# CompVis/zigma

Hardware: NVIDIA H100
Metric: denoiser tokens/s (bs*L*evals/s), zigzag8_b1, Euler sampling loop (higher is better)
Workload: dtype bf16

## Files before the change

include/zigma_b200.h:

```cpp
#ifndef ZIGMA_B200_H
#define ZIGMA_B200_H

#include <stdint.h>

#ifdef __cplusplus
extern "C" {
#endif

enum { ZG_F32 = 0, ZG_F16 = 1, ZG_BF16 = 2 };

enum {
    ZG_SCAN_DELTA_SOFTPLUS = 1,
    ZG_SCAN_VARIABLE_B = 2,
    ZG_SCAN_VARIABLE_C = 4,
    ZG_SCAN_OUT_REVERSE = 8,
    ZG_SCAN_OUT_ACCUMULATE = 16
};

int zg_abi_version(void);
const char *zg_last_error(void);
uint64_t zg_launch_count(void);
const char *zg_last_scan_kernel(void);
int zg_scan_kernel_choice(int64_t units16, int32_t sms, int32_t training_forward, int32_t *nd, int32_t *ns);

// ... 104 lines not shown
    const float *d_residual_out;
    const void *d_normed, *d_modded;
    const float *r, *rstd;
    const void *mix, *gate, *scale, *norm_w;
    const int32_t *rowmap;
    void *d_x, *d_mix;
    float *d_residual_in, *dgate, *dshift, *dscale, *d_norm_w;
    int64_t mod_rs;
    int32_t batch, seqlen, dim, dtype, nparts;
} zg_block_tail_bwd_params;

int zg_block_tail_bwd(const zg_block_tail_bwd_params *p, void *stream);

int64_t zg_selective_scan_bwd_det_workspace_bytes(const zg_scan_bwd_params *p);
int zg_selective_scan_bwd_det(const zg_scan_bwd_params *p, void *workspace, int64_t workspace_bytes, void *stream);
int64_t zg_causal_conv1d_bwd_det_workspace_bytes(const zg_conv_bwd_params *p);
int zg_causal_conv1d_bwd_det(const zg_conv_bwd_params *p, void *workspace, int64_t workspace_bytes, void *stream);
int64_t zg_add_norm_bwd_det_workspace_bytes(const zg_norm_bwd_params *p);
int zg_add_norm_bwd_det(const zg_norm_bwd_params *p, void *workspace, int64_t workspace_bytes, void *stream);
int64_t zg_block_tail_bwd_det_workspace_bytes(const zg_block_tail_bwd_params *p);
int zg_block_tail_bwd_det(const zg_block_tail_bwd_params *p, void *workspace, int64_t workspace_bytes, void *stream);

typedef struct {
    zg_block_tail_params base;
    const void *path_scale;
} zg_block_tail_dp_params;

typedef struct {
    zg_block_tail_bwd_params base;
    const void *path_scale;
} zg_block_tail_bwd_dp_params;

int zg_block_tail_fwd_dp(const zg_block_tail_dp_params *p, void *stream);
int zg_block_tail_bwd_dp(const zg_block_tail_bwd_dp_params *p, void *stream);
int64_t zg_block_tail_bwd_dp_det_workspace_bytes(const zg_block_tail_bwd_dp_params *p);
int zg_block_tail_bwd_dp_det(const zg_block_tail_bwd_dp_params *p, void *workspace, int64_t workspace_bytes, void *stream);

typedef struct {
    const void *q, *k, *v;
    void *o;
    float *lse;
    int64_t q_sb, q_rs, k_sb, k_rs, v_sb, v_rs, o_sb, o_rs;
    int32_t batch, L, Lk, heads, dim, dtype;
} zg_xattn_params;

int zg_cross_attn_fwd(const zg_xattn_params *p, void *stream);

typedef struct {
    zg_xattn_params fwd;
    const void *dout;
    void *dq, *dk, *dv;
    int64_t dout_sb, dout_rs, dq_sb, dq_rs, dk_sb, dk_rs, dv_sb, dv_rs;
    int32_t sms;
} zg_xattn_bwd_params;

int64_t zg_cross_attn_bwd_workspace_bytes(const zg_xattn_bwd_params *p);
int zg_cross_attn_bwd(const zg_xattn_bwd_params *p, void *workspace, int64_t workspace_bytes, void *stream);

typedef struct {
    const void *A, *B, *bias;
    void *C;
    const int32_t *out_rowmap;
    int64_t lda, ldb, ldc;
    int32_t M, N, K, rows_per_batch;
} zg_gemm_params;

// ... 44 lines not shown
```

zigma_b200/_lib.py:

```python
import ctypes as C
import os

import torch

_HERE = os.path.dirname(os.path.abspath(__file__))
LIB_PATH = os.environ.get("ZIGMA_B200_LIB") or os.path.join(_HERE, "lib", "libzigma_b200.so")

ZG_F32, ZG_F16, ZG_BF16 = 0, 1, 2
SCAN_DELTA_SOFTPLUS, SCAN_VARIABLE_B, SCAN_VARIABLE_C, SCAN_OUT_REVERSE, SCAN_OUT_ACCUMULATE = 1, 2, 4, 8, 16
_DT = {torch.float32: ZG_F32, torch.float16: ZG_F16, torch.bfloat16: ZG_BF16}

vp, i64, i32, f32 = C.c_void_p, C.c_int64, C.c_int32, C.c_float


class ScanParams(C.Structure):
    _fields_ = ([(n, vp) for n in ("u", "delta", "z", "B", "C", "A", "D", "delta_bias", "z_rowmap", "out", "last_state", "ckpt")]
                + [(n, i64) for n in ("u_sb", "u_sd", "u_sl", "delta_sb", "delta_sd", "delta_sl", "z_sb", "z_sd", "z_sl",
                                      "out_sb", "out_sd", "out_sl", "B_sb", "B_sg", "B_sn", "B_sl", "C_sb", "C_sg", "C_sn", "C_sl")]
                + [(n, i32) for n in ("batch", "dim", "seqlen", "dstate", "ngroups", "dtype", "flags", "ckpt_every")]
                + [(n, vp) for n in ("dt_w", "dt_x")]
                + [(n, i64) for n in ("dt_w_ld", "dt_x_sb", "dt_x_sl")]
                + [(n, i32) for n in ("dt_rank", "z_batch_inner")]
                + [("z_sbi", i64)])

# ... 25 lines not shown
                + [(n, i64) for n in ("x_rs", "res_rs", "y_rs", "resout_rs")]
                + [(n, i32) for n in ("nrows", "ncols", "dtype", "res_dtype", "wdtype", "is_rms")]
                + [("eps", f32)])


class NormBwdParams(C.Structure):
    _fields_ = ([(n, vp) for n in ("dy", "dresidual", "x", "weight", "mean", "rstd", "dx", "dresidual_in", "dweight", "dbias")]
                + [(n, i64) for n in ("dy_rs", "dres_rs", "x_rs", "dx_rs", "dresin_rs")]
                + [(n, i32) for n in ("nrows", "ncols", "dtype", "res_dtype", "wdtype", "is_rms")])


class BlockTailParams(C.Structure):
    _fields_ = ([(n, vp) for n in ("x", "mix", "gate", "shift", "scale", "norm_w", "residual", "rowmap", "residual_out", "normed", "modded")]
                + [("mod_rs", i64)]
                + [(n, i32) for n in ("batch", "seqlen", "dim", "dtype", "final_layer")]
                + [("eps", f32), ("rstd", vp)])


class BlockTailBwdParams(C.Structure):
    _fields_ = ([(n, vp) for n in ("d_residual_out", "d_normed", "d_modded", "r", "rstd", "mix", "gate", "scale", "norm_w", "rowmap",
                                   "d_x", "d_mix", "d_residual_in", "dgate", "dshift", "dscale", "d_norm_w")]
                + [("mod_rs", i64)]
                + [(n, i32) for n in ("batch", "seqlen", "dim", "dtype", "nparts")])


class BlockTailDpParams(C.Structure):
    _fields_ = [("base", BlockTailParams), ("path_scale", vp)]


class BlockTailBwdDpParams(C.Structure):
    _fields_ = [("base", BlockTailBwdParams), ("path_scale", vp)]


class XattnParams(C.Structure):
    _fields_ = ([(n, vp) for n in ("q", "k", "v", "o", "lse")]
                + [(n, i64) for n in ("q_sb", "q_rs", "k_sb", "k_rs", "v_sb", "v_rs", "o_sb", "o_rs")]
                + [(n, i32) for n in ("batch", "L", "Lk", "heads", "dim", "dtype")])


class XattnBwdParams(C.Structure):
    _fields_ = ([("fwd", XattnParams)]
                + [(n, vp) for n in ("dout", "dq", "dk", "dv")]
                + [(n, i64) for n in ("dout_sb", "dout_rs", "dq_sb", "dq_rs", "dk_sb", "dk_rs", "dv_sb", "dv_rs")]
                + [("sms", i32)])


class TextPrologueParams(C.Structure):
    _fields_ = ([(n, vp) for n in ("x", "mix", "gate", "shift", "scale", "rowmap", "hidden", "q_in", "mean", "rstd")]
                + [("mod_rs", i64)]
                + [(n, i32) for n in ("batch", "seqlen", "dim", "dtype")]
                + [("eps", f32)])


class TextPrologueBwdParams(C.Structure):
    _fields_ = ([(n, vp) for n in ("d_hidden", "d_q", "hidden", "mix", "gate", "scale", "mean", "rstd", "rowmap", "d_x", "d_mix",
                                   "dgate", "dshift", "dscale")]
                + [("mod_rs", i64)]
                + [(n, i32) for n in ("batch", "seqlen", "dim", "dtype", "nparts")])


class GemmParams(C.Structure):
    _fields_ = ([(n, vp) for n in ("A", "B", "bias", "C", "out_rowmap")]
                + [(n, i64) for n in ("lda", "ldb", "ldc")]
                + [(n, i32) for n in ("M", "N", "K", "rows_per_batch")])


class AdamWParams(C.Structure):
    _fields_ = ([(n, vp) for n in ("param", "exp_avg", "exp_avg_sq", "ema", "grad", "grad_scale_ptr")]
                + [("n", i64)]
                + [(n, f32) for n in ("lr", "beta1", "beta2", "eps", "weight_decay", "bias_correction1", "bias_correction2",
                                      "ema_decay", "grad_scale")])


EXPORTS = ["zg_abi_version", "zg_last_error", "zg_launch_count", "zg_last_scan_kernel", "zg_scan_kernel_choice", "zg_selective_scan_fwd", "zg_selective_scan_bwd",
           "zg_causal_conv1d_fwd", "zg_causal_conv1d_bwd", "zg_add_norm_fwd", "zg_add_norm_bwd",
           "zg_block_tail_fwd", "zg_block_tail_fwd_pe", "zg_block_tail_bwd", "zg_block_tail_fwd_dp", "zg_block_tail_bwd_dp",
           "zg_gemm_bf16_tn", "zg_adamw_ema_step", "zg_text_prologue_fwd", "zg_text_prologue_bwd"]
DET_OPS = ["zg_selective_scan_bwd", "zg_causal_conv1d_bwd", "zg_add_norm_bwd", "zg_block_tail_bwd", "zg_block_tail_bwd_dp",
           "zg_text_prologue_bwd"]
EXPORTS += [n + s for n in DET_OPS for s in ("_det", "_det_workspace_bytes")]
EXPORTS += ["zg_cross_attn_fwd", "zg_cross_attn_bwd", "zg_cross_attn_bwd_workspace_bytes"]

_lib = None


def lib():
    global _lib
    if _lib is None:
        if not os.path.exists(LIB_PATH):
            raise RuntimeError(
                f"zigma_b200: native library {LIB_PATH} not found -- build it with "
                f"`python -c 'import __graft_entry__ as g; g.build()'` (nvcc, sm_90a). There is no CPU/PyTorch fallback.")
        l = C.CDLL(LIB_PATH)
        l.zg_last_error.restype = C.c_char_p
        l.zg_launch_count.restype = C.c_uint64
        l.zg_last_scan_kernel.restype = C.c_char_p
        l.zg_last_scan_kernel.argtypes = []
        l.zg_scan_kernel_choice.restype = C.c_int
        l.zg_scan_kernel_choice.argtypes = [C.c_int64, C.c_int32, C.c_int32, C.POINTER(C.c_int32), C.POINTER(C.c_int32)]
        for name in EXPORTS[5:]:
            if name.endswith("_det_workspace_bytes"):
                getattr(l, name).restype = C.c_int64
                getattr(l, name).argtypes = [C.c_void_p]
            elif name.endswith("_det"):
                getattr(l, name).restype = C.c_int
                getattr(l, name).argtypes = [C.c_void_p, C.c_void_p, C.c_int64, C.c_void_p]
            else:
                getattr(l, name).restype = C.c_int
                getattr(l, name).argtypes = [C.c_void_p, C.c_void_p]
# ... 61 lines not shown
```

zigma_b200/csrc/norm.cu:

```cuda
#include "zg_common.cuh"
#include <stdlib.h>

namespace zg {

__device__ __forceinline__ float ld_dt(const void *p, int64_t i, int dt) {
    if (dt == ZG_F32) return reinterpret_cast<const float *>(p)[i];
    if (dt == ZG_F16) return __half2float(reinterpret_cast<const __half *>(p)[i]);
    return __bfloat162float(reinterpret_cast<const __nv_bfloat16 *>(p)[i]);
}
__device__ __forceinline__ void st_dt(void *p, int64_t i, int dt, float v) {
    if (dt == ZG_F32) reinterpret_cast<float *>(p)[i] = v;
    else if (dt == ZG_F16) reinterpret_cast<__half *>(p)[i] = __float2half_rn(v);
    else reinterpret_cast<__nv_bfloat16 *>(p)[i] = __float2bfloat16_rn(v);
}
template <typename T> __device__ __forceinline__ float round_to(float v) { return zg_to_float<T>(zg_from_float<T>(v)); }

template <typename T> __device__ __forceinline__ void ld4(const T *p, int64_t i, float (&o)[4]);
template <> __device__ __forceinline__ void ld4<float>(const float *p, int64_t i, float (&o)[4]) {
    float4 v = *reinterpret_cast<const float4 *>(p + i);
    o[0] = v.x; o[1] = v.y; o[2] = v.z; o[3] = v.w;
}
template <> __device__ __forceinline__ void ld4<__nv_bfloat16>(const __nv_bfloat16 *p, int64_t i, float (&o)[4]) {
    uint2 v = *reinterpret_cast<const uint2 *>(p + i);
    o[0] = __uint_as_float(v.x << 16); o[1] = __uint_as_float(v.x & 0xffff0000u);
// ... 342 lines not shown
            if (q < nq) {
                float o[4];
#pragma unroll
                for (int i = 0; i < 4; ++i) o[i] = (r[k][i] - mean) * rstd2;
                st4<T>(normed, 4 * q, o);
            }
        }
        return;
    }
#pragma unroll
    for (int k = 0; k < MAXQ; ++k) {
        const int q = lane + 32 * k;
        if (q < nq) {
            st4<T>(normed, 4 * q, r[k]);
            if (modded) {
                float sc[4], sh[4], o[4];
                ld4<T>(scale, 4 * q, sc);
                ld4<T>(shift, 4 * q, sh);
#pragma unroll
                for (int i = 0; i < 4; ++i)
                    o[i] = round_to<T>(r[k][i] * round_to<T>(1.f + sc[i])) + sh[i];
                st4<T>(modded, 4 * q, o);
            }
        }
    }
}

#ifndef ZG_TAIL_PREFETCH_MOD
#define ZG_TAIL_PREFETCH_MOD 1
#endif
#ifndef ZG_TAIL_MINB
#define ZG_TAIL_MINB 12
#endif
template <typename T, int MAXQ, bool PE, bool DP>
__device__ __forceinline__ void block_tail_row4_body(const zg_block_tail_params &p, const void *path_scale) {
    __shared__ float red[3][4];
    const int64_t row = blockIdx.x;
    const int tid = threadIdx.x, lane = tid & 31, warp = tid >> 5;
    const int D = p.dim, nq = D >> 2;
    const int b = (int)(row / p.seqlen), l = (int)(row % p.seqlen);
    const T *x = reinterpret_cast<const T *>(p.x) + row * D;
    const T *mix = nullptr;
    if (p.mix) {
        const int64_t src = (PE ? 0 : (int64_t)b * p.seqlen) + (p.rowmap ? p.rowmap[l] : l);
        mix = reinterpret_cast<const T *>(p.mix) + src * D;
    }
    const T *gate = (!PE && p.gate) ? reinterpret_cast<const T *>(p.gate) + (int64_t)b * p.mod_rs : nullptr;
    const T *shift = p.shift ? reinterpret_cast<const T *>(p.shift) + (int64_t)b * p.mod_rs : nullptr;
    const T *scale = p.scale ? reinterpret_cast<const T *>(p.scale) + (int64_t)b * p.mod_rs : nullptr;
    const T *nw = reinterpret_cast<const T *>(p.norm_w);
    const float *res = p.residual ? p.residual + row * D : nullptr;
    float *rout = p.residual_out ? p.residual_out + row * D : nullptr;
    T *normed = reinterpret_cast<T *>(p.normed) + row * D;
    T *modded = p.modded ? reinterpret_cast<T *>(p.modded) + row * D : nullptr;
    auto block_sum = [&](float v, int slot) {
        v = zg_warp_sum(v);
        if (lane == 0) red[slot][warp] = v;
        __syncthreads();
        return (red[slot][0] + red[slot][1]) + (red[slot][2] + red[slot][3]);
    };

    Raw4<T> rx[MAXQ], rm[MAXQ], rg[MAXQ], rw[MAXQ];
#if ZG_TAIL_PREFETCH_MOD
    Raw4<T> rsc[MAXQ], rsh[MAXQ];
#endif
    float4 rr[MAXQ];
#pragma unroll
    for (int k = 0; k < MAXQ; ++k) {
        const int q = tid + 128 * k;
        if (q < nq) {
            rx[k] = ldraw<T>(x, 4 * q);
            if (mix) { rm[k] = ldraw<T>(mix, 4 * q); rg[k] = PE ? raw_ones<T>() : ldraw<T>(gate, 4 * q); }
            if (res) rr[k] = *reinterpret_cast<const float4 *>(res + 4 * q);
            rw[k] = ldraw<T>(nw, 4 * q);
#if ZG_TAIL_PREFETCH_MOD
            if (modded) { rsc[k] = ldraw<T>(scale, 4 * q); rsh[k] = ldraw<T>(shift, 4 * q); }
#endif
        }
    }
    float dps = 1.f;
    if constexpr (DP) dps = zg_to_float<T>(reinterpret_cast<const T *>(path_scale)[b]);
    float r[MAXQ][4];
    float sumsq = 0.f;
#pragma unroll
    for (int k = 0; k < MAXQ; ++k) {
        const int q = tid + 128 * k;
        if (q < nq) {
            cvt4<T>(rx[k], r[k]);
            if (mix) {
                float m[4], g[4];
                cvt4<T>(rm[k], m);
                cvt4<T>(rg[k], g);
#pragma unroll
                for (int i = 0; i < 4; ++i)
                    r[k][i] = round_to<T>(r[k][i] + round_to<T>(g[i] * m[i]));
            }
            if constexpr (DP) {
#pragma unroll
                for (int i = 0; i < 4; ++i) r[k][i] = round_to<T>(__fmul_rn(r[k][i], dps));
            }
            if (res) {
                r[k][0] += rr[k].x; r[k][1] += rr[k].y; r[k][2] += rr[k].z; r[k][3] += rr[k].w;
            }
            if (rout) st4<float>(rout, 4 * q, r[k]);
#pragma unroll
            for (int i = 0; i < 4; ++i) sumsq += r[k][i] * r[k][i];
        }
    }
    const float rstd = 1.f / sqrtf(block_sum(sumsq, 0) / D + p.eps);
    if (p.rstd && tid == 0) p.rstd[row] = rstd;
    float sum2 = 0.f;
#pragma unroll
    for (int k = 0; k < MAXQ; ++k) {
        const int q = tid + 128 * k;
        if (q < nq) {
            float w[4];
            cvt4<T>(rw[k], w);
#pragma unroll
            for (int i = 0; i < 4; ++i) {
                r[k][i] = round_to<T>(r[k][i] * rstd * w[i]);
                sum2 += r[k][i];
            }
        }
    }
    if (!DP && p.final_layer) {
        const float mean = block_sum(sum2, 1) / D;
        float s2 = 0.f;
#pragma unroll
        for (int k = 0; k < MAXQ; ++k)
            if (tid + 128 * k < nq)
#pragma unroll
                for (int i = 0; i < 4; ++i) { const float d = r[k][i] - mean; s2 += d * d; }
        const float rstd2 = 1.f / sqrtf(block_sum(s2, 2) / D + 1e-6f);
#pragma unroll
        for (int k = 0; k < MAXQ; ++k) {
            const int q = tid + 128 * k;
            if (q < nq) {
                float o[4];
#pragma unroll
                for (int i = 0; i < 4; ++i) o[i] = (r[k][i] - mean) * rstd2;
                st4<T>(normed, 4 * q, o);
            }
        }
        return;
    }
#pragma unroll
    for (int k = 0; k < MAXQ; ++k) {
        const int q = tid + 128 * k;
        if (q < nq) {
            st4<T>(normed, 4 * q, r[k]);
            if (modded) {
                float sc[4], sh[4], o[4];
#if ZG_TAIL_PREFETCH_MOD
                cvt4<T>(rsc[k], sc);
                cvt4<T>(rsh[k], sh);
#else
                ld4<T>(scale, 4 * q, sc);
                ld4<T>(shift, 4 * q, sh);
#endif
#pragma unroll
                for (int i = 0; i < 4; ++i)
                    o[i] = round_to<T>(r[k][i] * round_to<T>(1.f + sc[i])) + sh[i];
                st4<T>(modded, 4 * q, o);
            }
        }
    }
}

template <typename T, int MAXQ, bool PE>
__global__ void __launch_bounds__(128, ZG_TAIL_MINB) block_tail_row4_kernel(const zg_block_tail_params p) {
    block_tail_row4_body<T, MAXQ, PE, false>(p, nullptr);
}

template <typename T, int MAXQ>
__global__ void __launch_bounds__(128, ZG_TAIL_MINB) block_tail_dp_fwd_kernel(const zg_block_tail_dp_params p) {
    block_tail_row4_body<T, MAXQ, false, true>(p.base, p.path_scale);
}

template <typename T> static int block_tail_dp_t(const zg_block_tail_dp_params &p, cudaStream_t s) {
    const unsigned g4 = (unsigned)((int64_t)p.base.batch * p.base.seqlen);
    if (p.base.dim <= 512) block_tail_dp_fwd_kernel<T, 1><<<g4, 128, 0, s>>>(p);
    else block_tail_dp_fwd_kernel<T, 2><<<g4, 128, 0, s>>>(p);
    zg_count_launch();
    return zg_check_launch("block_tail_fwd_dp");
}

template <typename T> static int block_tail_t(const zg_block_tail_params &p, cudaStream_t s, bool pe = false) {
    const int64_t nrows = (int64_t)p.batch * p.seqlen;
    static int row4 = -1;
    if (row4 < 0) { const char *e = getenv("ZG_TAIL_ROW4"); row4 = e ? atoi(e) : 1; }
    if ((row4 || pe) && nrows <= 0x7fffffffLL && p.dim <= 2048) {
        const unsigned g4 = (unsigned)nrows;
#define ZG_TAIL4(Q) do { if (pe) block_tail_row4_kernel<T, Q, true><<<g4, 128, 0, s>>>(p); else block_tail_row4_kernel<T, Q, false><<<g4, 128, 0, s>>>(p); } while (0)
        if (p.dim <= 512) ZG_TAIL4(1);
        else if (p.dim <= 1024) ZG_TAIL4(2);
        else if (p.dim <= 1536) ZG_TAIL4(3);
        else ZG_TAIL4(4);
#undef ZG_TAIL4
        zg_count_launch();
        return zg_check_launch("block_tail_fwd");
    }
    if (pe) return zg_set_error("block_tail_fwd_pe: dim <= 2048 and fewer than 2^31 rows only, got dim %d", p.dim);
    const unsigned grid = (unsigned)((nrows * 32 + 127) / 128);
    if (p.dim <= 512) block_tail_kernel<T, 4><<<grid, 128, 0, s>>>(p);
    else if (p.dim <= 640) block_tail_kernel<T, 5><<<grid, 128, 0, s>>>(p);
    else if (p.dim <= 768) block_tail_kernel<T, 6><<<grid, 128, 0, s>>>(p);
    else if (p.dim <= 1024) block_tail_kernel<T, 8><<<grid, 128, 0, s>>>(p);
    else if (p.dim <= 1536) block_tail_kernel<T, 12><<<grid, 128, 0, s>>>(p);
    else block_tail_kernel<T, NORM_MAXQ><<<grid, 128, 0, s>>>(p);
// ... 345 lines not shown
    if (pp->nrows == 0) return 0;
    return norm_bwd_dispatch<false>(*pp, (cudaStream_t)stream);
}

static ZgDetLayout norm_bwd_det_layout(const zg_norm_bwd_params &p, void *ws) {
    ZgDetLayout lay;
    lay.ws = static_cast<unsigned char *>(ws);
    if (p.nrows <= 0 || p.ncols <= 0) return lay;
    const int64_t rows = (int64_t)zg::norm_bwd_grid(p) * (zg::norm_bwd_vec(p) ? 1 : 4);
    lay.add(p.dweight, rows, p.ncols);
    lay.add(p.dbias, rows, p.ncols);
    return lay;
}

extern "C" int64_t zg_add_norm_bwd_det_workspace_bytes(const zg_norm_bwd_params *p) {
    return p ? norm_bwd_det_layout(*p, nullptr).bytes : 0;
}

extern "C" int zg_add_norm_bwd_det(const zg_norm_bwd_params *pp, void *workspace, int64_t workspace_bytes, void *stream) {
    ZG_REQUIRE(pp != nullptr, "add_norm_bwd_det: null params");
    if (int rc = norm_bwd_validate(*pp)) return rc;
    if (pp->nrows == 0) return 0;
    const ZgDetLayout lay = norm_bwd_det_layout(*pp, workspace);
    ZG_REQUIRE_WORKSPACE(lay, workspace, workspace_bytes, "add_norm_bwd_det");
    zg_norm_bwd_params p = *pp;
    int i = 0;
    if (p.dweight) p.dweight = lay.reg[i++].part;
    if (p.dbias) p.dbias = lay.reg[i++].part;
    cudaStream_t s = (cudaStream_t)stream;
    if (int rc = norm_bwd_dispatch<true>(p, s)) return rc;
    return lay.reduce(s);
}

static int block_tail_fwd_validate(const zg_block_tail_params &p, bool pe) {
    ZG_REQUIRE(p.x && p.norm_w && p.normed, "block_tail_fwd: null tensor pointer");
    if (pe) ZG_REQUIRE(p.mix && !p.gate && !p.rowmap && !p.residual, "block_tail_fwd_pe: takes the (seqlen, dim) table as mix and no gate / rowmap / residual");
    else ZG_REQUIRE(!p.mix || p.gate, "block_tail_fwd: mix needs gate");
    ZG_REQUIRE(!p.modded || (p.shift && p.scale), "block_tail_fwd: modded needs shift and scale");
    ZG_REQUIRE(p.dim > 0 && p.dim % 4 == 0 && p.dim <= 4 * 32 * zg::NORM_MAXQ, "block_tail_fwd: dim must be a multiple of 4 and <= %d, got %d",
               4 * 32 * zg::NORM_MAXQ, p.dim);
    ZG_REQUIRE(p.mod_rs % 4 == 0, "block_tail_fwd: modulation row stride must be a multiple of 4");
    ZG_REQUIRE(aligned16(p.x) && aligned16(p.mix) && aligned16(p.residual) && aligned16(p.residual_out) && aligned16(p.normed) && aligned16(p.modded),
               "block_tail_fwd: row tensors must be 16-byte aligned");
    ZG_REQUIRE(aligned_quad(p.gate, p.dtype) && aligned_quad(p.shift, p.dtype) && aligned_quad(p.scale, p.dtype) && aligned_quad(p.norm_w, p.dtype),
               "block_tail_fwd: gate / shift / scale / norm_w must be aligned to 4 elements");
    return 0;
}

static int block_tail_fwd_entry(const zg_block_tail_params *pp, void *stream, bool pe) {
    ZG_REQUIRE(pp != nullptr, "block_tail_fwd: null params");
    const zg_block_tail_params &p = *pp;
    if (int rc = block_tail_fwd_validate(p, pe)) return rc;
    const int64_t nrows = (int64_t)p.batch * p.seqlen;
    if (nrows == 0) return 0;
    cudaStream_t s = (cudaStream_t)stream;
    switch (p.dtype) {
        case ZG_F32: return zg::block_tail_t<float>(p, s, pe);
        case ZG_F16: return zg::block_tail_t<__half>(p, s, pe);
        case ZG_BF16: return zg::block_tail_t<__nv_bfloat16>(p, s, pe);
    }
    return zg_set_error("block_tail_fwd: bad dtype %d", p.dtype);
}

extern "C" int zg_block_tail_fwd(const zg_block_tail_params *pp, void *stream) { return block_tail_fwd_entry(pp, stream, false); }
extern "C" int zg_block_tail_fwd_pe(const zg_block_tail_params *pp, void *stream) { return block_tail_fwd_entry(pp, stream, true); }

static bool aligned_elem(const void *p, int dtype) {
    return (reinterpret_cast<uintptr_t>(p) & ((dtype == ZG_F32 ? sizeof(float) : sizeof(__half)) - 1)) == 0;
}

extern "C" int zg_block_tail_fwd_dp(const zg_block_tail_dp_params *pp, void *stream) {
    ZG_REQUIRE(pp != nullptr, "block_tail_fwd_dp: null params");
    const zg_block_tail_params &p = pp->base;
    ZG_REQUIRE(pp->path_scale != nullptr, "block_tail_fwd_dp: null path_scale");
    ZG_REQUIRE(p.residual != nullptr && p.mix != nullptr, "block_tail_fwd_dp: needs residual and mix (the first block has no drop path)");
    ZG_REQUIRE(p.final_layer == 0, "block_tail_fwd_dp: final_layer is not supported");
    ZG_REQUIRE(p.dim <= 1024, "block_tail_fwd_dp: dim must be <= 1024, got %d", p.dim);
    if (int rc = block_tail_fwd_validate(p, false)) return rc;
    ZG_REQUIRE(aligned_elem(pp->path_scale, p.dtype), "block_tail_fwd_dp: path_scale must be aligned to its element size");
    const int64_t nrows = (int64_t)p.batch * p.seqlen;
    if (nrows == 0) return 0;
    ZG_REQUIRE(nrows <= 0x7fffffffLL, "block_tail_fwd_dp: fewer than 2^31 rows only");
    cudaStream_t s = (cudaStream_t)stream;
    switch (p.dtype) {
        case ZG_F32: return zg::block_tail_dp_t<float>(*pp, s);
        case ZG_F16: return zg::block_tail_dp_t<__half>(*pp, s);
        case ZG_BF16: return zg::block_tail_dp_t<__nv_bfloat16>(*pp, s);
    }
    return zg_set_error("block_tail_fwd_dp: bad dtype %d", p.dtype);
}

static int block_tail_bwd_validate(const zg_block_tail_bwd_params &p) {
    ZG_REQUIRE(p.r && p.rstd && p.norm_w && p.d_x, "block_tail_bwd: null tensor pointer");
    ZG_REQUIRE((p.mix != nullptr) == (p.gate != nullptr) && (p.mix != nullptr) == (p.d_mix != nullptr), "block_tail_bwd: mix, gate and d_mix go together");
    ZG_REQUIRE(!p.d_modded || p.scale, "block_tail_bwd: d_modded needs scale");
    ZG_REQUIRE(p.dim > 0 && p.dim % 4 == 0 && p.dim <= 1024, "block_tail_bwd: dim must be a multiple of 4 and <= 1024, got %d", p.dim);
    ZG_REQUIRE(p.mod_rs % 4 == 0, "block_tail_bwd: modulation row stride must be a multiple of 4");
    ZG_REQUIRE(p.nparts >= 1 && p.nparts <= 65535, "block_tail_bwd: nparts (rows of the d_norm_w partials buffer = CTAs) must be in [1, 65535]");
    ZG_REQUIRE(p.dtype == ZG_F32 || p.dtype == ZG_F16 || p.dtype == ZG_BF16, "block_tail_bwd: bad dtype %d", p.dtype);
    ZG_REQUIRE(aligned16(p.r) && aligned16(p.d_residual_out) && aligned16(p.d_normed) && aligned16(p.d_modded) && aligned16(p.mix) && aligned16(p.d_x) &&
                   aligned16(p.d_mix) && aligned16(p.d_residual_in),
// ... 170 lines not shown
```

zigma_b200/csrc/scan_fwd_wp2.cuh:

```cuda
#pragma once
#include "scan_fwd_wp.cuh"

namespace zg {

constexpr int WP2_CH = 32;
constexpr int WP2_MAX_WARPS = 9;

struct Wp2Layout {
    static constexpr int NSTAGE = 3;
    static constexpr int TILE = PT_TL * WP2_CH * 2;
    static constexpr int RAW = 3 * TILE + PT_TL * 64;
    static constexpr int DDU_ROW = WP2_CH * 8;
    static constexpr int DDU_OFF = NSTAGE * RAW;
    static constexpr int BCF_OFF = DDU_OFF + PT_TL * DDU_ROW;
    static constexpr int BAR_OFF = BCF_OFF + PT_TL * 32 * 4;
    static constexpr int WARP_BYTES = ((BAR_OFF + NSTAGE * 8 + 127) / 128) * 128;
};

template <int PITCH>
__device__ __forceinline__ void wp2_main_stage(const unsigned char *__restrict__ ddu_j, const float *__restrict__ bq, unsigned char *__restrict__ ypart,
                                               zg_f2 (&h)[2][4], const zg_f2 (&Al)[2][4]) {
    auto decay = [&](float dlx, const zg_f2 (&al)[4], zg_f2 (&a)[4]) {
        const zg_f2 dl = zg_splat2(dlx);
#pragma unroll
        for (int q = 0; q < 4; ++q) a[q] = zg_ex2_mufu2(zg_mul2(dl, al[q]));
    };
    zg_f2 a0[4], a1[4];
    float4 dd = *reinterpret_cast<const float4 *>(ddu_j);
    decay(dd.x, Al[0], a0);
    decay(dd.z, Al[1], a1);
#pragma unroll
    for (int t = 0; t < PT_TL; ++t) {
        const float4 *bc = reinterpret_cast<const float4 *>(bq + t * 16);
        zg_f2 Bp[4], Cp[4];
#pragma unroll
        for (int k = 0; k < 2; ++k) {
            const float4 Bk = bc[32 * k], Ck = bc[2 + 32 * k];
            Bp[2 * k] = make_float2(Bk.x, Bk.y); Bp[2 * k + 1] = make_float2(Bk.z, Bk.w);
            Cp[2 * k] = make_float2(Ck.x, Ck.y); Cp[2 * k + 1] = make_float2(Ck.z, Ck.w);
// ... 143 lines not shown
    int slot = 0, nslot = 1;
    uint32_t npar = 0;
    for (int s = 0; s < nstages; ++s) {
        wp2_main_stage<LY::DDU_ROW>(ddu_j, bq, ypart, h2, Al2p);
        const unsigned char *raw = smem + slot * LY::RAW;
        __syncwarp();
        if (s + 1 < nstages) {
            const unsigned char *rawn = smem + nslot * LY::RAW;
            zg_mbar_wait(&full[nslot], npar);
#pragma unroll
            for (int k = 0; k < NITEM; ++k) { post_item(k, raw); pre_item(k, rawn); }
            bc_convert(rawn);
        } else {
#pragma unroll
            for (int k = 0; k < NITEM; ++k) post_item(k, raw);
        }
        gout += out_stage;
        __syncwarp();
        issue_stage(slot);
        slot = nslot;
        if (++nslot == NSTAGE) { nslot = 0; npar ^= 1; }
    }
    if (p.last_state) {
#pragma unroll
        for (int c = 0; c < 2; ++c) {
            float4 *dst = reinterpret_cast<float4 *>(p.last_state + ((int64_t)b * E + e + c) * 16 + 8 * part);
            dst[0] = make_float4(h2[c][0].x, h2[c][0].y, h2[c][1].x, h2[c][1].y);
            dst[1] = make_float4(h2[c][2].x, h2[c][2].y, h2[c][3].x, h2[c][3].y);
        }
    }
}

template <typename T, bool PLAIN>
__global__ void __launch_bounds__(32 * WP2_MAX_WARPS, 2) scan_fwd_wp2_kernel(const zg_scan_params p) {
    extern __shared__ __align__(1024) unsigned char smem_all[];
    const int lane = threadIdx.x & 31;
    const int warp = __shfl_sync(0xffffffffu, (int)(threadIdx.x >> 5), 0);
    const int per_group = p.dim / p.ngroups;
    const int units_per_group = per_group / WP2_CH;
    const int units = units_per_group * p.ngroups;
    const int wu = blockIdx.x * (int)(blockDim.x >> 5) + warp;
    if (wu >= units * p.batch) return;
    const int unit = wu % units;
    wp2_body<T, PLAIN>(p, smem_all + warp * Wp2Layout::WARP_BYTES, lane, wu / units, unit / units_per_group, unit * WP2_CH);
}

inline int wp2_pick_warps(long long units, int sms) {
    if (units > 18LL * sms) return 3;
    const long long per_sm = (units + sms - 1) / sms;
    const int ctas_per_sm = per_sm > 4 ? 2 : 1;
    return (int)((units + (long long)sms * ctas_per_sm - 1) / ((long long)sms * ctas_per_sm));
}

template <typename T, bool PLAIN> int wp2_launch(const zg_scan_params &p, cudaStream_t stream) {
    using LY = Wp2Layout;
    auto kern = scan_fwd_wp2_kernel<T, PLAIN>;
    static bool attr_dev[64] = {};
    static int sms_dev[64] = {};
    int dev = 0;
    cudaGetDevice(&dev);
    if (!attr_dev[dev & 63]) {
        cudaError_t err = cudaFuncSetAttribute(kern, cudaFuncAttributeMaxDynamicSharedMemorySize, WP2_MAX_WARPS * LY::WARP_BYTES);
        if (err != cudaSuccess) return zg_set_error("scan_fwd(wp2): cudaFuncSetAttribute(%d B smem): %s", WP2_MAX_WARPS * LY::WARP_BYTES, cudaGetErrorString(err));
        cudaFuncSetAttribute(kern, cudaFuncAttributePreferredSharedMemoryCarveout, cudaSharedmemCarveoutMaxShared);
        cudaDeviceGetAttribute(&sms_dev[dev & 63], cudaDevAttrMultiProcessorCount, dev);
        attr_dev[dev & 63] = true;
    }
    const long long units = (long long)(p.dim / WP2_CH) * p.batch;
    const int w = wp2_pick_warps(units, sms_dev[dev & 63] > 0 ? sms_dev[dev & 63] : 132);
    const long long nblk = (units + w - 1) / w;
    kern<<<(unsigned)nblk, 32 * w, w * LY::WARP_BYTES, stream>>>(p);
    zg_count_launch();
    zg_note_scan_kernel("zg::scan_fwd_wp2_kernel (warp-private pipeline, 32 channels per warp, cp.async)");
    return zg_check_launch("scan_fwd(wp2)");
}

template <typename T> int wp2_launch_variant(const zg_scan_params &p, cudaStream_t stream) {
    const bool plain = p.z && (p.flags & ZG_SCAN_DELTA_SOFTPLUS) && !(p.flags & (ZG_SCAN_OUT_REVERSE | ZG_SCAN_OUT_ACCUMULATE));
    return plain ? wp2_launch<T, true>(p, stream) : wp2_launch<T, false>(p, stream);
}

}
```

zigma_b200/engine.py:

```python
import os

import torch
import torch.nn.functional as F

from . import _lib
from .causal_conv1d_interface import _conv_fwd
from .selective_scan_interface import _scan_fwd


def _i32(t):
    return t.to(torch.int32).contiguous()


def _linear(x2d, weight, bias=None):
    if x2d.dtype == torch.bfloat16 and os.environ.get("ZIGMA_TCGEN05", "1") == "1" and x2d.stride(0) % 8 == 0 and weight.stride(0) % 8 == 0:
        from .gemm import linear_bf16
        return linear_bf16(x2d, weight, bias)
    return F.linear(x2d, weight, bias)


def fused_dt_ok(dtype, E, L, N, R, dt_w):
    return (dtype in (torch.bfloat16, torch.float16) and N == 16 and R in (40, 48) and L % 8 == 0 and E % 64 == 0
            and dt_w.dtype == dtype and dt_w.stride(1) == 1 and dt_w.stride(0) % 8 == 0 and (R + 2 * N) % 8 == 0)


def scan_hot_path_ok(dtype, E, L, N, R):
    return (dtype in (torch.bfloat16, torch.float16) and N == 16 and L % 8 == 0 and L > 0 and E % 64 == 0 and R % 8 == 0
            and (R + 2 * N) % 8 == 0 and os.environ.get("ZG_SCAN_TMA", "1") != "0")


def block_tail(x, mix, gate, shift, scale, norm_w, residual, rowmap, eps, final=False, mod_div=1, want_modded=True, want_rstd=False,
               mix_bcast=False, path_scale=None):
    _lib.require_cuda(x, mix, gate, shift, scale, norm_w, residual, rowmap, path_scale)
    if path_scale is not None and (path_scale.dtype != x.dtype or tuple(path_scale.shape) != (x.shape[0],) or not path_scale.is_contiguous()):
        raise RuntimeError(f"block_tail: path_scale must be a contiguous ({x.shape[0]},) tensor in {x.dtype}, got "
                           f"{tuple(path_scale.shape)} {path_scale.dtype}")
    Bt, L, D = x.shape
    if mod_div != 1:
        gate = None if gate is None else gate.repeat_interleave(mod_div, dim=0)
        shift = None if shift is None else shift.repeat_interleave(mod_div, dim=0)
        scale = None if scale is None else scale.repeat_interleave(mod_div, dim=0)
    mods = [m for m in (gate, shift, scale) if m is not None]
    rs = mods[0].stride(0) if mods else 0
    for m in mods:
        if m.stride(0) != rs or m.stride(1) != 1:
            raise RuntimeError("block_tail: modulation views must share one row stride")
    if norm_w.dtype != x.dtype:
        norm_w = norm_w.to(x.dtype)
    def _as_x(t):
        return t if (t is None or t.dtype == x.dtype) else t.to(x.dtype)
    mix = _as_x(mix)
    if mix is not None and not mix.is_contiguous():
        mix = mix.contiguous()
    if any(m is not None and m.dtype != x.dtype for m in (gate, shift, scale)):
        D_ = x.shape[-1]
        packed = torch.zeros((x.shape[0] // mod_div if mod_div != 1 else x.shape[0], 3 * D_), dtype=x.dtype, device=x.device)
        for i_, m in enumerate((gate, shift, scale)):
            if m is not None:
                packed[:, i_ * D_:(i_ + 1) * D_] = m
        gate = None if gate is None else packed[:, :D_]
        shift = None if shift is None else packed[:, D_:2 * D_]
        scale = None if scale is None else packed[:, 2 * D_:]
    if residual is not None and residual.dtype != torch.float32:
        raise RuntimeError("block_tail: the residual stream must be fp32 (residual_in_fp32=True)")
    res_out = torch.empty((Bt, L, D), dtype=torch.float32, device=x.device) if not final else None
    normed = torch.empty_like(x)
    modded = torch.empty_like(x) if (want_modded and not final) else None
    p = _lib.BlockTailParams()
    p.x, p.mix, p.gate, p.shift, p.scale = _lib.ptr(x), _lib.ptr(mix), _lib.ptr(gate), _lib.ptr(shift), _lib.ptr(scale)
    p.norm_w, p.residual, p.rowmap = _lib.ptr(norm_w), _lib.ptr(residual), _lib.ptr(rowmap)
    p.residual_out, p.normed, p.modded = _lib.ptr(res_out), _lib.ptr(normed), _lib.ptr(modded)
    p.mod_rs = rs
    p.batch, p.seqlen, p.dim = Bt, L, D
    p.dtype, p.final_layer, p.eps = _lib.dt(x), int(final), float(eps)
    rstd = torch.empty((Bt * L,), dtype=torch.float32, device=x.device) if want_rstd else None
    p.rstd = _lib.ptr(rstd)
    if mix_bcast and (mix is None or mix.numel() != L * D or gate is not None or rowmap is not None or residual is not None):
        raise RuntimeError("block_tail: mix_bcast takes a (seqlen, dim) mix table and no gate / rowmap / residual")
    if path_scale is not None:
        _lib.call("zg_block_tail_fwd_dp", _lib.BlockTailDpParams(p, _lib.ptr(path_scale)))
    else:
        _lib.call("zg_block_tail_fwd_pe" if mix_bcast else "zg_block_tail_fwd", p)
    if want_rstd:
        return res_out, normed, modded, rstd
    return res_out, normed, modded


def text_prologue(x, mix, gate, shift, scale, rowmap, eps, mod_div=1, want_stats=False):
    _lib.require_cuda(x, mix, gate, shift, scale, rowmap)
    Bt, L, D = x.shape
    if mod_div != 1:
        gate, shift, scale = (m.repeat_interleave(mod_div, dim=0) for m in (gate, shift, scale))
    if any(t.dtype != x.dtype for t in (mix, gate, shift, scale)) or tuple(mix.shape) != (Bt, L, D) or not mix.is_contiguous():
        raise RuntimeError("text_prologue: mix must be a contiguous tensor of x's shape and every operand in x's dtype")
    rs = gate.stride(0)
    if any(m.stride(0) != rs or m.stride(1) != 1 or tuple(m.shape) != (Bt, D) for m in (gate, shift, scale)):
        raise RuntimeError("text_prologue: gate / shift / scale must be (batch, dim) views sharing one row stride")
    hidden, q_in = torch.empty_like(x), torch.empty_like(x)
    mean = torch.empty((Bt * L,), dtype=torch.float32, device=x.device) if want_stats else None
    rstd = torch.empty((Bt * L,), dtype=torch.float32, device=x.device) if want_stats else None
    p = _lib.TextPrologueParams()
    p.x, p.mix, p.gate, p.shift, p.scale, p.rowmap = _lib.ptr(x), _lib.ptr(mix), _lib.ptr(gate), _lib.ptr(shift), _lib.ptr(scale), _lib.ptr(rowmap)
    p.hidden, p.q_in, p.mean, p.rstd = _lib.ptr(hidden), _lib.ptr(q_in), _lib.ptr(mean), _lib.ptr(rstd)
    p.mod_rs = rs
    p.batch, p.seqlen, p.dim, p.dtype, p.eps = Bt, L, D, _lib.dt(x), float(eps)
    _lib.call("zg_text_prologue_fwd", p)
    if want_stats:
        return hidden, q_in, mean, rstd
    return hidden, q_in


class ZigMaEngine:
# ... 157 lines not shown
                y = self._core(xz, B * T, K, lay, lay["fwd"], lay["perm"])
                mix = _linear(y.reshape(B * T * K, E), lay["out_proj"], lay["out_bias"]).view(B * T, K, D)
                return mix, lay["perm_rev"], T
            if self._temporal_fused_ok(xz.dtype, lay, T, K):
                tb = self._temporal_tables(lay, T, K, xz.device)
                y = self._core_temporal(xz, B, T, K, lay, lay["fwd"], tb)
                mix = _linear(y.reshape(B * L, E), lay["out_proj"], lay["out_bias"]).view(B, L, D)
                return mix, tb["out"], 1
            xz_t = xz.view(B, T, K, 2 * E).permute(0, 2, 1, 3).reshape(B * K * T, 2 * E)
            y = self._core(xz_t, B * K, T, lay, lay["fwd"], lay["perm"])
            mix = _linear(y.reshape(B * K * T, E), lay["out_proj"], lay["out_bias"]).view(B * K, T, D)
            mix = mix[:, lay["perm_rev64"], :].reshape(B, K, T, D).permute(0, 2, 1, 3).reshape(B, L, D)
            return mix, None, 1
        mix = _linear(y.reshape(B * L, E), lay["out_proj"], lay["out_bias"]).view(B, L, D)
        return mix, rowmap, 1

    def _forward_impl(self, x, t, y):
        m = self.m
        tokens = self._patch_embed(x)
        pe = None
        if (tokens is not None and m.use_pe in (1, 2) and not (m.video_frames > 0 and m.tpe) and m.pos_embed.dtype == tokens.dtype
                and tokens.shape[-1] <= 2048 and os.environ.get("ZIGMA_FOLD_PE", "1") != "0"):
            pe = m.pos_embed.detach().reshape(-1, m.pos_embed.shape[-1]).contiguous()
        hs, c, text = m.embed(x, t, y, tokens=tokens, add_pos=pe is None)
        hs = hs.contiguous()
        B, L, D = hs.shape
        if pe is not None and pe.shape[0] != L:
            raise RuntimeError(f"pos_embed has {pe.shape[0]} rows, the model {L} tokens")
        depth = len(self.layers)
        nmod = 6 if m.has_text else 3
        mods = _linear(F.silu(c), self.ada_w, self.ada_b).view(B, depth, nmod, D)
        eps = m.blocks[0].norm.eps
        lay0 = self.layers[0]
        residual, normed, modded = block_tail(hs, pe, None, mods[:, 0, 0], mods[:, 0, 1], lay0["norm_w"], None, None, eps,
                                              mix_bcast=pe is not None)
        for i, lay in enumerate(self.layers):
            mix, rowmap, fold = self._mixer(modded, lay)
            last = i == depth - 1
            nw = m.norm_f.weight if last else self.layers[i + 1]["norm_w"]
            neps = m.norm_f.eps if last else m.blocks[i + 1].norm.eps
            gate = mods[:, i, 2]
            shift = None if last else mods[:, i + 1, 0]
            scale = None if last else mods[:, i + 1, 1]
            if m.has_text:
                blk = m.blocks[i]
                Bf = B * fold
                hidden, q_in = text_prologue(normed.view(Bf, L // fold, D), mix.view(Bf, L // fold, D), gate, mods[:, i, 3], mods[:, i, 4],
                                             rowmap, blk.norm_msa.eps, mod_div=fold)
                fold = 1
                mix, rowmap, gate, normed = blk.msa(q_in.view(B, L, D), text=text, mask=None).contiguous(), None, mods[:, i, 5], hidden.view(B, L, D)
            if fold != 1:
                Bf = B * fold
                residual, normed, modded = block_tail(normed.view(Bf, L // fold, D), mix, gate, shift, scale, nw,
                                                      residual.view(Bf, L // fold, D), rowmap, neps, final=last, mod_div=fold)
                normed = normed.view(B, L, D)
                if not last:
                    residual, modded = residual.view(B, L, D), modded.view(B, L, D)
            else:
                residual, normed, modded = block_tail(normed, mix, gate, shift, scale, nw, residual, rowmap, neps, final=last)
        out = _linear(normed.reshape(B * L, D), m.final_layer.linear.weight, m.final_layer.linear.bias).view(B, L, -1)
        if m.video_frames > 0:
            return m.unpatchify_video(out, m.video_frames)
        return m.unpatchify(out)

    @torch.no_grad()
    def forward(self, x, t, y=None):
        if self._versions != self._param_versions():
            self.refresh()
        if not self.use_graph:
            return self._forward_impl(x, t, y)
        key = (tuple(x.shape), x.dtype, tuple(t.shape), t.dtype, None if y is None else (tuple(y.shape), y.dtype))
        g = self._graphs.get(key)
        if g is None:
            sx, st_, sy = x.clone(), t.clone(), None if y is None else y.clone()
            s = torch.cuda.Stream()
            s.wait_stream(torch.cuda.current_stream())
            with torch.cuda.stream(s):
                for _ in range(2):
                    self._forward_impl(sx, st_, sy)
            torch.cuda.current_stream().wait_stream(s)
            graph = torch.cuda.CUDAGraph()
            with torch.cuda.graph(graph):
                sout = self._forward_impl(sx, st_, sy)
            g = (graph, sx, st_, sy, sout)
            self._graphs[key] = g
        graph, sx, st_, sy, sout = g
        sx.copy_(x)
        st_.copy_(t)
        if y is not None:
            sy.copy_(y)
        graph.replay()
        return sout.clone()
# ... 53 lines not shown
```

Measured before the change: 2.166 million.

## Rebuild normed input from residual and rstd in block tail; widen scan warps

Adds a block-tail variant that recomputes the previous layer's normed activations from the fp32 residual, the per-row rstd and the norm weight, instead of writing and re-reading a bf16 normed tensor. Intermediate normed outputs are no longer stored, which removes one activation write and read per layer. Separately, the wp2 scan kernel now allows up to 20 warps per CTA with one CTA per SM, and the warp-count heuristic changes to match, spreading small workloads across more warps. The cost is an extra rstd write per row and some recompute work, plus different occupancy and register limits in the scan kernel.

```diff
diff --git a/include/zigma_b200.h b/include/zigma_b200.h
--- a/include/zigma_b200.h
+++ b/include/zigma_b200.h
@@ -160,6 +160,14 @@
 } zg_block_tail_bwd_dp_params;
 
 int zg_block_tail_fwd_dp(const zg_block_tail_dp_params *p, void *stream);
+
+typedef struct {
+    zg_block_tail_params base;
+    const float *x_rstd;
+    const void *x_norm_w;
+} zg_block_tail_rebuild_params;
+
+int zg_block_tail_fwd_rebuild(const zg_block_tail_rebuild_params *p, void *stream);
 int zg_block_tail_bwd_dp(const zg_block_tail_bwd_dp_params *p, void *stream);
 int64_t zg_block_tail_bwd_dp_det_workspace_bytes(const zg_block_tail_bwd_dp_params *p);
 int zg_block_tail_bwd_dp_det(const zg_block_tail_bwd_dp_params *p, void *workspace, int64_t workspace_bytes, void *stream);
diff --git a/zigma_b200/_lib.py b/zigma_b200/_lib.py
--- a/zigma_b200/_lib.py
+++ b/zigma_b200/_lib.py
@@ -81,6 +81,10 @@
     _fields_ = [("base", BlockTailBwdParams), ("path_scale", vp)]
 
 
+class BlockTailRebuildParams(C.Structure):
+    _fields_ = [("base", BlockTailParams), ("x_rstd", vp), ("x_norm_w", vp)]
+
+
 class XattnParams(C.Structure):
     _fields_ = ([(n, vp) for n in ("q", "k", "v", "o", "lse")]
                 + [(n, i64) for n in ("q_sb", "q_rs", "k_sb", "k_rs", "v_sb", "v_rs", "o_sb", "o_rs")]
@@ -124,6 +128,7 @@
 EXPORTS = ["zg_abi_version", "zg_last_error", "zg_launch_count", "zg_last_scan_kernel", "zg_scan_kernel_choice", "zg_selective_scan_fwd", "zg_selective_scan_bwd",
            "zg_causal_conv1d_fwd", "zg_causal_conv1d_bwd", "zg_add_norm_fwd", "zg_add_norm_bwd",
            "zg_block_tail_fwd", "zg_block_tail_fwd_pe", "zg_block_tail_bwd", "zg_block_tail_fwd_dp", "zg_block_tail_bwd_dp",
+           "zg_block_tail_fwd_rebuild",
            "zg_gemm_bf16_tn", "zg_adamw_ema_step", "zg_text_prologue_fwd", "zg_text_prologue_bwd"]
 DET_OPS = ["zg_selective_scan_bwd", "zg_causal_conv1d_bwd", "zg_add_norm_bwd", "zg_block_tail_bwd", "zg_block_tail_bwd_dp",
            "zg_text_prologue_bwd"]
diff --git a/zigma_b200/csrc/norm.cu b/zigma_b200/csrc/norm.cu
--- a/zigma_b200/csrc/norm.cu
+++ b/zigma_b200/csrc/norm.cu
@@ -398,14 +398,15 @@
 #ifndef ZG_TAIL_MINB
 #define ZG_TAIL_MINB 12
 #endif
-template <typename T, int MAXQ, bool PE, bool DP>
-__device__ __forceinline__ void block_tail_row4_body(const zg_block_tail_params &p, const void *path_scale) {
+template <typename T, int MAXQ, bool PE, bool DP, bool RB = false>
+__device__ __forceinline__ void block_tail_row4_body(const zg_block_tail_params &p, const void *path_scale, const float *x_rstd = nullptr,
+                                                     const void *x_norm_w = nullptr) {
     __shared__ float red[3][4];
     const int64_t row = blockIdx.x;
     const int tid = threadIdx.x, lane = tid & 31, warp = tid >> 5;
     const int D = p.dim, nq = D >> 2;
     const int b = (int)(row / p.seqlen), l = (int)(row % p.seqlen);
-    const T *x = reinterpret_cast<const T *>(p.x) + row * D;
+    const T *x = RB ? reinterpret_cast<const T *>(x_norm_w) : reinterpret_cast<const T *>(p.x) + row * D;
     const T *mix = nullptr;
     if (p.mix) {
         const int64_t src = (PE ? 0 : (int64_t)b * p.seqlen) + (p.rowmap ? p.rowmap[l] : l);
@@ -437,22 +438,32 @@
         if (q < nq) {
             rx[k] = ldraw<T>(x, 4 * q);
             if (mix) { rm[k] = ldraw<T>(mix, 4 * q); rg[k] = PE ? raw_ones<T>() : ldraw<T>(gate, 4 * q); }
-            if (res) rr[k] = *reinterpret_cast<const float4 *>(res + 4 * q);
+            if (RB || res) rr[k] = *reinterpret_cast<const float4 *>(res + 4 * q);
             rw[k] = ldraw<T>(nw, 4 * q);
 #if ZG_TAIL_PREFETCH_MOD
-            if (modded) { rsc[k] = ldraw<T>(scale, 4 * q); rsh[k] = ldraw<T>(shift, 4 * q); }
+            if (!RB && modded) { rsc[k] = ldraw<T>(scale, 4 * q); rsh[k] = ldraw<T>(shift, 4 * q); }
 #endif
         }
     }
     float dps = 1.f;
     if constexpr (DP) dps = zg_to_float<T>(reinterpret_cast<const T *>(path_scale)[b]);
+    float xrs = 0.f;
+    if constexpr (RB) xrs = x_rstd[row];
     float r[MAXQ][4];
     float sumsq = 0.f;
 #pragma unroll
     for (int k = 0; k < MAXQ; ++k) {
         const int q = tid + 128 * k;
         if (q < nq) {
-            cvt4<T>(rx[k], r[k]);
+            if constexpr (RB) {
+                float w[4];
+                const float rp[4] = {rr[k].x, rr[k].y, rr[k].z, rr[k].w};
+                cvt4<T>(rx[k], w);
+#pragma unroll
+                for (int i = 0; i < 4; ++i) r[k][i] = round_to<T>(__fmul_rn(__fmul_rn(rp[i], xrs), w[i]));
+            } else {
+                cvt4<T>(rx[k], r[k]);
+            }
             if (mix) {
                 float m[4], g[4];
                 cvt4<T>(rm[k], m);
@@ -465,7 +476,7 @@
 #pragma unroll
                 for (int i = 0; i < 4; ++i) r[k][i] = round_to<T>(__fmul_rn(r[k][i], dps));
             }
-            if (res) {
+            if (RB || res) {
                 r[k][0] += rr[k].x; r[k][1] += rr[k].y; r[k][2] += rr[k].z; r[k][3] += rr[k].w;
             }
             if (rout) st4<float>(rout, 4 * q, r[k]);
@@ -514,12 +525,17 @@
     for (int k = 0; k < MAXQ; ++k) {
         const int q = tid + 128 * k;
         if (q < nq) {
-            st4<T>(normed, 4 * q, r[k]);
+            if (!RB || p.normed) st4<T>(normed, 4 * q, r[k]);
             if (modded) {
                 float sc[4], sh[4], o[4];
 #if ZG_TAIL_PREFETCH_MOD
-                cvt4<T>(rsc[k], sc);
-                cvt4<T>(rsh[k], sh);
+                if constexpr (RB) {
+                    ld4<T>(scale, 4 * q, sc);
+                    ld4<T>(shift, 4 * q, sh);
+                } else {
+                    cvt4<T>(rsc[k], sc);
+                    cvt4<T>(rsh[k], sh);
+                }
 #else
                 ld4<T>(scale, 4 * q, sc);
                 ld4<T>(shift, 4 * q, sh);
@@ -541,6 +557,19 @@
 template <typename T, int MAXQ>
 __global__ void __launch_bounds__(128, ZG_TAIL_MINB) block_tail_dp_fwd_kernel(const zg_block_tail_dp_params p) {
     block_tail_row4_body<T, MAXQ, false, true>(p.base, p.path_scale);
+}
+
+template <typename T, int MAXQ>
+__global__ void __launch_bounds__(128, ZG_TAIL_MINB) block_tail_rebuild_fwd_kernel(const zg_block_tail_rebuild_params p) {
+    block_tail_row4_body<T, MAXQ, false, false, true>(p.base, nullptr, p.x_rstd, p.x_norm_w);
+}
+
+template <typename T> static int block_tail_rebuild_t(const zg_block_tail_rebuild_params &p, cudaStream_t s) {
+    const unsigned g4 = (unsigned)((int64_t)p.base.batch * p.base.seqlen);
+    if (p.base.dim <= 512) block_tail_rebuild_fwd_kernel<T, 1><<<g4, 128, 0, s>>>(p);
+    else block_tail_rebuild_fwd_kernel<T, 2><<<g4, 128, 0, s>>>(p);
+    zg_count_launch();
+    return zg_check_launch("block_tail_fwd_rebuild");
 }
 
 template <typename T> static int block_tail_dp_t(const zg_block_tail_dp_params &p, cudaStream_t s) {
@@ -952,8 +981,8 @@
     return lay.reduce(s);
 }
 
-static int block_tail_fwd_validate(const zg_block_tail_params &p, bool pe) {
-    ZG_REQUIRE(p.x && p.norm_w && p.normed, "block_tail_fwd: null tensor pointer");
+static int block_tail_fwd_validate(const zg_block_tail_params &p, bool pe, bool rebuild = false) {
+    ZG_REQUIRE((rebuild || (p.x && p.normed)) && p.norm_w, "block_tail_fwd: null tensor pointer");
     if (pe) ZG_REQUIRE(p.mix && !p.gate && !p.rowmap && !p.residual, "block_tail_fwd_pe: takes the (seqlen, dim) table as mix and no gate / rowmap / residual");
     else ZG_REQUIRE(!p.mix || p.gate, "block_tail_fwd: mix needs gate");
     ZG_REQUIRE(!p.modded || (p.shift && p.scale), "block_tail_fwd: modded needs shift and scale");
@@ -987,6 +1016,28 @@
 
 static bool aligned_elem(const void *p, int dtype) {
     return (reinterpret_cast<uintptr_t>(p) & ((dtype == ZG_F32 ? sizeof(float) : sizeof(__half)) - 1)) == 0;
+}
+
+extern "C" int zg_block_tail_fwd_rebuild(const zg_block_tail_rebuild_params *pp, void *stream) {
+    ZG_REQUIRE(pp != nullptr, "block_tail_fwd_rebuild: null params");
+    const zg_block_tail_params &p = pp->base;
+    ZG_REQUIRE(p.x == nullptr, "block_tail_fwd_rebuild: x must be NULL (it is rebuilt from residual, x_rstd and x_norm_w)");
+    ZG_REQUIRE(p.residual && pp->x_rstd && pp->x_norm_w, "block_tail_fwd_rebuild: needs residual, x_rstd and x_norm_w");
+    ZG_REQUIRE(p.normed || !p.final_layer, "block_tail_fwd_rebuild: final_layer needs normed");
+    ZG_REQUIRE(p.dim <= 1024, "block_tail_fwd_rebuild: dim must be <= 1024, got %d", p.dim);
+    if (int rc = block_tail_fwd_validate(p, false, true)) return rc;
+    ZG_REQUIRE(aligned_quad(pp->x_norm_w, p.dtype) && (reinterpret_cast<uintptr_t>(pp->x_rstd) & 3) == 0,
+               "block_tail_fwd_rebuild: x_norm_w must be aligned to 4 elements, x_rstd to 4 bytes");
+    const int64_t nrows = (int64_t)p.batch * p.seqlen;
+    if (nrows == 0) return 0;
+    ZG_REQUIRE(nrows <= 0x7fffffffLL, "block_tail_fwd_rebuild: fewer than 2^31 rows only");
+    cudaStream_t s = (cudaStream_t)stream;
+    switch (p.dtype) {
+        case ZG_F32: return zg::block_tail_rebuild_t<float>(*pp, s);
+        case ZG_F16: return zg::block_tail_rebuild_t<__half>(*pp, s);
+        case ZG_BF16: return zg::block_tail_rebuild_t<__nv_bfloat16>(*pp, s);
+    }
+    return zg_set_error("block_tail_fwd_rebuild: bad dtype %d", p.dtype);
 }
 
 extern "C" int zg_block_tail_fwd_dp(const zg_block_tail_dp_params *pp, void *stream) {
diff --git a/zigma_b200/csrc/scan_fwd_wp2.cuh b/zigma_b200/csrc/scan_fwd_wp2.cuh
--- a/zigma_b200/csrc/scan_fwd_wp2.cuh
+++ b/zigma_b200/csrc/scan_fwd_wp2.cuh
@@ -4,7 +4,7 @@
 namespace zg {
 
 constexpr int WP2_CH = 32;
-constexpr int WP2_MAX_WARPS = 9;
+constexpr int WP2_MAX_WARPS = 20;
 
 struct Wp2Layout {
     static constexpr int NSTAGE = 3;
@@ -214,7 +214,7 @@
 }
 
 template <typename T, bool PLAIN>
-__global__ void __launch_bounds__(32 * WP2_MAX_WARPS, 2) scan_fwd_wp2_kernel(const zg_scan_params p) {
+__global__ void __launch_bounds__(32 * WP2_MAX_WARPS, 1) scan_fwd_wp2_kernel(const zg_scan_params p) {
     extern __shared__ __align__(1024) unsigned char smem_all[];
     const int lane = threadIdx.x & 31;
     const int warp = __shfl_sync(0xffffffffu, (int)(threadIdx.x >> 5), 0);
@@ -228,10 +228,8 @@
 }
 
 inline int wp2_pick_warps(long long units, int sms) {
-    if (units > 18LL * sms) return 3;
-    const long long per_sm = (units + sms - 1) / sms;
-    const int ctas_per_sm = per_sm > 4 ? 2 : 1;
-    return (int)((units + (long long)sms * ctas_per_sm - 1) / ((long long)sms * ctas_per_sm));
+    if (units > (long long)WP2_MAX_WARPS * sms) return 3;
+    return (int)((units + sms - 1) / sms);
 }
 
 template <typename T, bool PLAIN> int wp2_launch(const zg_scan_params &p, cudaStream_t stream) {
diff --git a/zigma_b200/engine.py b/zigma_b200/engine.py
--- a/zigma_b200/engine.py
+++ b/zigma_b200/engine.py
@@ -30,12 +30,23 @@
 
 
 def block_tail(x, mix, gate, shift, scale, norm_w, residual, rowmap, eps, final=False, mod_div=1, want_modded=True, want_rstd=False,
-               mix_bcast=False, path_scale=None):
+               mix_bcast=False, path_scale=None, x_from=None):
     _lib.require_cuda(x, mix, gate, shift, scale, norm_w, residual, rowmap, path_scale)
-    if path_scale is not None and (path_scale.dtype != x.dtype or tuple(path_scale.shape) != (x.shape[0],) or not path_scale.is_contiguous()):
-        raise RuntimeError(f"block_tail: path_scale must be a contiguous ({x.shape[0]},) tensor in {x.dtype}, got "
+    if (x is None) != (x_from is not None) or (x_from is not None and (residual is None or path_scale is not None or mix_bcast)):
+        raise RuntimeError("block_tail: x_from replaces x, needs the residual and takes no path_scale / mix_bcast")
+    if x_from is not None:
+        x_rstd, x_norm_w = x_from
+        _lib.require_cuda(x_rstd, x_norm_w)
+        xdt, xdev = x_norm_w.dtype, residual.device
+        Bt, L, D = residual.shape
+        if x_rstd.dtype != torch.float32 or x_rstd.numel() != Bt * L or not x_rstd.is_contiguous() or x_norm_w.numel() != D:
+            raise RuntimeError("block_tail: x_from needs the previous tail's (Bt * L,) fp32 rstd and its (D,) norm_w")
+    else:
+        xdt, xdev = x.dtype, x.device
+        Bt, L, D = x.shape
+    if path_scale is not None and (path_scale.dtype != xdt or tuple(path_scale.shape) != (Bt,) or not path_scale.is_contiguous()):
+        raise RuntimeError(f"block_tail: path_scale must be a contiguous ({Bt},) tensor in {xdt}, got "
                            f"{tuple(path_scale.shape)} {path_scale.dtype}")
-    Bt, L, D = x.shape
     if mod_div != 1:
         gate = None if gate is None else gate.repeat_interleave(mod_div, dim=0)
         shift = None if shift is None else shift.repeat_interleave(mod_div, dim=0)
@@ -45,16 +56,16 @@
     for m in mods:
         if m.stride(0) != rs or m.stride(1) != 1:
             raise RuntimeError("block_tail: modulation views must share one row stride")
-    if norm_w.dtype != x.dtype:
-        norm_w = norm_w.to(x.dtype)
+    if norm_w.dtype != xdt:
+        norm_w = norm_w.to(xdt)
     def _as_x(t):
-        return t if (t is None or t.dtype == x.dtype) else t.to(x.dtype)
+        return t if (t is None or t.dtype == xdt) else t.to(xdt)
     mix = _as_x(mix)
     if mix is not None and not mix.is_contiguous():
         mix = mix.contiguous()
-    if any(m is not None and m.dtype != x.dtype for m in (gate, shift, scale)):
-        D_ = x.shape[-1]
-        packed = torch.zeros((x.shape[0] // mod_div if mod_div != 1 else x.shape[0], 3 * D_), dtype=x.dtype, device=x.device)
+    if any(m is not None and m.dtype != xdt for m in (gate, shift, scale)):
+        D_ = D
+        packed = torch.zeros((Bt // mod_div if mod_div != 1 else Bt, 3 * D_), dtype=xdt, device=xdev)
         for i_, m in enumerate((gate, shift, scale)):
             if m is not None:
                 packed[:, i_ * D_:(i_ + 1) * D_] = m
@@ -63,21 +74,23 @@
         scale = None if scale is None else packed[:, 2 * D_:]
     if residual is not None and residual.dtype != torch.float32:
         raise RuntimeError("block_tail: the residual stream must be fp32 (residual_in_fp32=True)")
-    res_out = torch.empty((Bt, L, D), dtype=torch.float32, device=x.device) if not final else None
-    normed = torch.empty_like(x)
-    modded = torch.empty_like(x) if (want_modded and not final) else None
+    res_out = torch.empty((Bt, L, D), dtype=torch.float32, device=xdev) if not final else None
+    normed = torch.empty((Bt, L, D), dtype=xdt, device=xdev) if (x_from is None or final) else None
+    modded = torch.empty((Bt, L, D), dtype=xdt, device=xdev) if (want_modded and not final) else None
     p = _lib.BlockTailParams()
     p.x, p.mix, p.gate, p.shift, p.scale = _lib.ptr(x), _lib.ptr(mix), _lib.ptr(gate), _lib.ptr(shift), _lib.ptr(scale)
     p.norm_w, p.residual, p.rowmap = _lib.ptr(norm_w), _lib.ptr(residual), _lib.ptr(rowmap)
     p.residual_out, p.normed, p.modded = _lib.ptr(res_out), _lib.ptr(normed), _lib.ptr(modded)
     p.mod_rs = rs
     p.batch, p.seqlen, p.dim = Bt, L, D
-    p.dtype, p.final_layer, p.eps = _lib.dt(x), int(final), float(eps)
-    rstd = torch.empty((Bt * L,), dtype=torch.float32, device=x.device) if want_rstd else None
+    p.dtype, p.final_layer, p.eps = _lib.dt(xdt), int(final), float(eps)
+    rstd = torch.empty((Bt * L,), dtype=torch.float32, device=xdev) if want_rstd else None
     p.rstd = _lib.ptr(rstd)
     if mix_bcast and (mix is None or mix.numel() != L * D or gate is not None or rowmap is not None or residual is not None):
         raise RuntimeError("block_tail: mix_bcast takes a (seqlen, dim) mix table and no gate / rowmap / residual")
-    if path_scale is not None:
+    if x_from is not None:
+        _lib.call("zg_block_tail_fwd_rebuild", _lib.BlockTailRebuildParams(p, _lib.ptr(x_rstd), _lib.ptr(x_norm_w)))
+    elif path_scale is not None:
         _lib.call("zg_block_tail_fwd_dp", _lib.BlockTailDpParams(p, _lib.ptr(path_scale)))
     else:
         _lib.call("zg_block_tail_fwd_pe" if mix_bcast else "zg_block_tail_fwd", p)
@@ -301,8 +314,10 @@
         mods = _linear(F.silu(c), self.ada_w, self.ada_b).view(B, depth, nmod, D)
         eps = m.blocks[0].norm.eps
         lay0 = self.layers[0]
-        residual, normed, modded = block_tail(hs, pe, None, mods[:, 0, 0], mods[:, 0, 1], lay0["norm_w"], None, None, eps,
-                                              mix_bcast=pe is not None)
+        rebuild = not m.has_text and D <= 1024
+        residual, normed, modded, *rstd = block_tail(hs, pe, None, mods[:, 0, 0], mods[:, 0, 1], lay0["norm_w"], None, None, eps,
+                                                     mix_bcast=pe is not None, want_rstd=rebuild)
+        prev_w = lay0["norm_w"]
         for i, lay in enumerate(self.layers):
             mix, rowmap, fold = self._mixer(modded, lay)
             last = i == depth - 1
@@ -318,15 +333,19 @@
                                              rowmap, blk.norm_msa.eps, mod_div=fold)
                 fold = 1
                 mix, rowmap, gate, normed = blk.msa(q_in.view(B, L, D), text=text, mask=None).contiguous(), None, mods[:, i, 5], hidden.view(B, L, D)
+            tail_x = dict(x_from=(rstd[0], prev_w.to(hs.dtype)), want_rstd=not last) if rebuild else {}
             if fold != 1:
                 Bf = B * fold
-                residual, normed, modded = block_tail(normed.view(Bf, L // fold, D), mix, gate, shift, scale, nw,
-                                                      residual.view(Bf, L // fold, D), rowmap, neps, final=last, mod_div=fold)
-                normed = normed.view(B, L, D)
+                residual, normed, modded, *rstd = block_tail(None if rebuild else normed.view(Bf, L // fold, D), mix, gate, shift, scale,
+                                                             nw, residual.view(Bf, L // fold, D), rowmap, neps, final=last, mod_div=fold,
+                                                             **tail_x)
+                normed = normed.view(B, L, D) if normed is not None else None
                 if not last:
                     residual, modded = residual.view(B, L, D), modded.view(B, L, D)
             else:
-                residual, normed, modded = block_tail(normed, mix, gate, shift, scale, nw, residual, rowmap, neps, final=last)
+                residual, normed, modded, *rstd = block_tail(None if rebuild else normed, mix, gate, shift, scale, nw, residual, rowmap,
+                                                             neps, final=last, **tail_x)
+            prev_w = nw
         out = _linear(normed.reshape(B * L, D), m.final_layer.linear.weight, m.final_layer.linear.bias).view(B, L, -1)
         if m.video_frames > 0:
             return m.unpatchify_video(out, m.video_frames)
```

Result: faster. 2.320 million (median of 6 runs) (+7.1%).
